# tier4/lidar_feature_extraction

Hardware: AMD Instinct MI355X
Metric: scans/sec (64-ring x 1800 synthetic scans, extraction hot path, inputs resident in HBM) (higher is better)
Workload: dtype f64

## Files before the change

lidar_feature_extraction_amd/csrc/lfx_kernels_unit.hpp:

```cpp
#pragma once

#include "lfx_kernels_common.hpp"

#pragma clang fp contract(off)

namespace lfx
{

enum { kBitLK, kBitJL, kBitJR, kBitA, kBitS, kBitSelE, kBitSelS, kUnitBitArrays };

template<int CH>
struct UnitLds
{
  static constexpr int kSpan = 64 * CH;
  static constexpr int kBitWords = 2 * (CH + 2);
  uint32_t bits[kUnitBitArrays][kBitWords];
  double r[kSpan];
  union {
    double c[kSpan + 2];
    float2 pxy[kSpan + 2];
  };
  static constexpr int kBaseDwords = (kSpan * 8 + (kSpan + 2) * 8 + kUnitBitArrays * kBitWords * 4) / 4;
  static constexpr int kMinPadDwords = 2 * (2 * CH - 2);
  static constexpr int kPadDwords = ((8 - kBaseDwords % 32) + 32) % 32 + (((8 - kBaseDwords % 32) + 32) % 32 < kMinPadDwords ? 32 : 0);
  uint32_t pad_[kPadDwords];
};
static_assert(sizeof(UnitLds<5>) % 128 == 32 && sizeof(UnitLds<3>) % 128 == 32 && sizeof(UnitLds<4>) % 128 == 32 &&
  sizeof(UnitLds<6>) % 128 == 32 && sizeof(UnitLds<12>) % 128 == 32, "slab stride");
static_assert(7 * 4 * sizeof(UnitLds<5>) <= 160 * 1024 && 6 * 4 * sizeof(UnitLds<6>) <= 160 * 1024 && 8 * 4 * sizeof(UnitLds<4>) <= 160 * 1024,
  "workgroups per CU the launch bounds count on");
#ifndef LFX_UNIT_WAVES_CH5
#define LFX_UNIT_WAVES_CH5 7
#endif
#ifndef LFX_LIBRARY_SQRT
#define LFX_LIBRARY_SQRT 0
#endif
#ifndef LFX_COS_BAND
#define LFX_COS_BAND 0x1p-20f
#endif
constexpr int unit_waves_per_simd(int ch, int variant = 0, bool xf = false)
{
  return ch > 6 ? 3 : (ch == 6 ? 5 : (ch == 5 ? (variant == 0 && !xf ? LFX_UNIT_WAVES_CH5 : 6) : (ch == 4 ? 7 : 8)));
}

#define LFX_WAVE_SYNC() \
  do { \
    __builtin_amdgcn_fence(__ATOMIC_RELEASE, "wavefront"); \
    __builtin_amdgcn_wave_barrier(); \
    __builtin_amdgcn_fence(__ATOMIC_ACQUIRE, "wavefront"); \
  } while (0)

template<int NW>
__device__ __forceinline__ void lds_window_f64(const double * first, double (&w)[NW])
{
  static_assert(NW <= 22, "extend the wait's operand list");
  const uint32_t addr = (uint32_t)reinterpret_cast<uintptr_t>(first);
#pragma unroll
  for (int i = 0; i < NW; i++) {
    asm volatile ("ds_read_b64 %0, %1 offset:%2" : "=v"(w[i]) : "v"(addr), "n"(8 * i));
  }
  if constexpr (NW == 2) {
    asm volatile ("s_waitcnt lgkmcnt(0)" : "+v"(w[0]), "+v"(w[1]));
  } else if constexpr (NW == 5) {
    asm volatile ("s_waitcnt lgkmcnt(0)" : "+v"(w[0]), "+v"(w[1]), "+v"(w[2]), "+v"(w[3]), "+v"(w[4]));
  } else if constexpr (NW == 11) {
// ... 84 lines not shown
    }
#undef LFX_WRITELANE
    static_assert(kUnitMaxChunks <= 12, "one case per chunk");
  }
};

template<int CH>
__device__ __forceinline__ void put_words(UnitLds<CH> & U, int arr, const WordVec & v, int lane)
{
  const uint32_t addr = (uint32_t)reinterpret_cast<uintptr_t>(&U.bits[arr][0]) + 8u * (uint32_t)lane;
  const uint64_t data = ((uint64_t)v.hi << 32) | v.lo;
  uint64_t saved;
  asm volatile ("s_mov_b64 %0, exec\n\ts_mov_b64 exec, %3\n\tds_write_b64 %1, %2\n\ts_mov_b64 exec, %0"
    : "=&s"(saved) : "v"(addr), "v"(data), "n"((1u << (CH + 2)) - 1u) : "memory");
}

template<int CH>
__device__ inline uint32_t get_win(const UnitLds<CH> & U, int arr, int k, const UnitWin & w)
{
  const u32_alias_t * b = reinterpret_cast<const u32_alias_t *>(&U.bits[arr][2 * k + w.ofs]);
  return __builtin_amdgcn_alignbit(b[1], b[0], w.sh);
}

template<int CH>
__device__ inline uint32_t get_win_at(const UnitLds<CH> & U, int arr, int first)
{
  const uint32_t bit = (uint32_t)(first + 64);
  const u32_alias_t * b = reinterpret_cast<const u32_alias_t *>(&U.bits[arr][bit >> 5]);
  return __builtin_amdgcn_alignbit(b[1], b[0], bit & 31u);
}

__device__ __forceinline__ uint32_t from_lane_below(uint32_t v) {return (uint32_t)__builtin_amdgcn_update_dpp(0, (int)v, 0x138, 0xF, 0xF, true);}
__device__ __forceinline__ uint32_t from_lane_above(uint32_t v) {return (uint32_t)__builtin_amdgcn_update_dpp(0, (int)v, 0x130, 0xF, 0xF, true);}

template<int CH, int PT>
__device__ __forceinline__ uint32_t row_frame(uint32_t own)
{
  static_assert(PT >= 1 && PT <= 2 * CH && (PT > CH ? 3 * CH + PT : 2 * CH + PT) <= 32,
    "the halo of a lane's positions must lie in the two lanes either side of it, the frame in one register");
  const uint32_t below = from_lane_below(own), above = from_lane_above(own);
  uint32_t f = (own << PT) | (above << (PT + CH));
  if constexpr (PT >= CH) {f |= below << (PT - CH);} else {f |= below >> (CH - PT);}
  if constexpr (PT > CH) {
    f |= from_lane_below(below) >> (2 * CH - PT);
    f |= from_lane_above(above) << (PT + 2 * CH);
  }
  return f;
}

template<int CH>
__device__ __forceinline__ uint32_t row_hits(uint32_t frame, const uint32_t (&mask)[CH])
{
  uint32_t h = 0;
#pragma unroll
  for (int d = 0; d < CH; d++) {
    const uint32_t t = frame & mask[d];
    h |= (t < 1u ? t : 1u) << d;
  }
  return h;
}

template<int CH> struct RowDiv { static constexpr uint32_t kShift = 18, kMul = ((1u << 18) + CH - 1) / CH; };
template<int CH> constexpr bool row_div_exact()
{
  for (uint32_t q = 0; q < 64u * CH; q++) {
    if (((q * RowDiv<CH>::kMul) >> RowDiv<CH>::kShift) != q / CH) {return false;}
// ... 61 lines not shown
struct OrgScan
{
  const uint8_t * __restrict__ pts;
  const uint32_t * __restrict__ scan_begin;
  uint32_t * __restrict__ ring_count_out;
  uint32_t R, r0, wave, drop_zero;
  const uint32_t * __restrict__ xform;
  const uint32_t * __restrict__ geom;
};

struct UnitGeom
{
  int N, b0, b1, o0, o1, g0, span, K, qb0, qb1, qo0, qo1, qlo, qhi;
};

__device__ inline UnitGeom unit_geometry(int N, int P, int B, int j, int b0, int b1)
{
  UnitGeom G;
  G.N = N; G.b0 = b0; G.b1 = b1;
  G.o0 = j == 0 ? 0 : b0; G.o1 = j == B - 1 ? N : b1;
  const int H = P + 1;
  G.g0 = G.o0 - H; G.span = G.o1 + H - G.g0;
  G.K = (G.span + 63) >> 6;
  G.qb0 = b0 - G.g0; G.qb1 = b1 - G.g0;
  G.qo0 = G.o0 - G.g0; G.qo1 = G.o1 - G.g0;
  G.qlo = G.g0 < 0 ? -G.g0 : 0;
  G.qhi = (N - G.g0) < G.span ? (N - G.g0) : G.span;
  return G;
}

template<int PT, int CH, bool DEF, bool ORG, bool XF, bool SIDX = false>
__device__ __forceinline__ uint32_t unit_core(
  const Params & prm, UnitLds<CH> & U, const UnitGeom & G, uint32_t dbg_flags, uint32_t s, uint32_t slot, int j,
  const float (&x)[CH], const float (&y)[CH], const float (&z)[CH], const uint32_t (&src)[CH],
  const UnitTables * __restrict__ tab, bool second_pass, const OrgScan & og, size_t off, uint32_t max_rings,
  uint32_t rec_lo, uint32_t rec_hi, uint32_t & n_edge, uint32_t & n_surface, const int lane)
{
  const int P = PT > 0 ? PT : prm.P, B = prm.B;
  (void)B;
  const int N = G.N, o0 = G.o0, o1 = G.o1, g0 = G.g0, span = G.span, K = G.K;
  const int qb0 = G.qb0, qb1 = G.qb1, qo0 = G.qo0, qo1 = G.qo1, qlo = G.qlo, qhi = G.qhi;
  (void)o0; (void)o1;
  const UnitWin W0{(uint32_t)(lane + 48) >> 5, (uint32_t)(lane + 16) & 31u};
  const UnitWin W1{(uint32_t)(lane + 49) >> 5, (uint32_t)(lane + 17) & 31u};
  constexpr uint32_t kOvrOccluded = 1u, kOvrRange = 2u, kOvrBeam = 4u;
  uint32_t ovr[(CH + 9) / 10];
#pragma unroll
  for (int t = 0; t < (CH + 9) / 10; t++) {ovr[t] = 0;}
  LFX_STAMP(2);
#pragma unroll
  for (int k = 0; k < CH; k++) {
    if (k < K) {
      const int q = 64 * k + lane;
      const double xd = (double)x[k], yd = (double)y[k];
      U.r[q] = sqrt_sum_of_squares(xd * xd + yd * yd);
    }
  }
  LFX_WAVE_SYNC();
  LFX_STAMP(3);
  {
    asm volatile ("" ::: "memory");
    const double dist_diff = DEF ? 0.3 : tab->prm.dist_diff;
    const double min_range = DEF ? 0.1 : tab->prm.min_range, max_range = DEF ? 100.0 : tab->prm.max_range;
    const double pb_ratio = DEF ? 0.02 : tab->prm.pb_ratio;
    const float pb_ratio_f = DEF ? 0.02f : tab->prm.pb_ratio_f;
    const double cos_bound = tab->prm.cos_bound;
    const int pair_end = qo1 < qhi - 1 ? qo1 : qhi - 1;
    uint64_t bad = 0;
    uint64_t zero_pair = 0;
    uint64_t prev_top = 0;
    WordVec vlk, vjl, vjr;
    const float cbf = tab->prm.cos_bound_f;
    const bool ratio_ok = pb_ratio_f >= 0x1p-9f;
    double c_dd = dist_diff, c_min = min_range, c_max = max_range;
    float c_one_lo = 1.0f - LFX_COS_BAND, c_one_hi = 1.0f + LFX_COS_BAND, c_tiny = 1e-18f, c_big = 1e30f, c_zero = 0.f, c_small = 1e-30f;
    asm volatile ("" : "+v"(c_dd), "+v"(c_min), "+v"(c_max), "+v"(c_one_lo), "+v"(c_one_hi), "+v"(c_tiny), "+v"(c_big), "+v"(c_zero), "+v"(c_small));
#pragma unroll
    for (int k = 0; k < CH; k++) {
      if (k < K) {
        const int q = 64 * k + lane;
        const uint64_t pair = in_span(q, qlo, qhi - 1);
        const float2 nb = U.pxy[q + 1];
        double rw3[3];
        lds_window_f64(&U.r[k == 0 ? (q > 0 ? q - 1 : 0) : q - 1], rw3);
        double rk = rw3[1], rn = rw3[2];
        const double rm = rw3[0];
        if (k == 0) {
          rk = q == 0 ? rw3[0] : rk;
          rn = q == 0 ? rw3[1] : rn;
        }
        zero_pair |= pair & in_span(q, qo0, qo1) & bal(rk == 0.) & bal(rn == 0.);
        {
          uint64_t spec;
          const uint64_t less = polar_less_masks(x[k], y[k], nb.x, nb.y, spec, c_tiny);
          bad |= in_span(q, qo0, pair_end) & (spec | ~less);
        }
        const float dotf = x[k] * nb.x + y[k] * nb.y;
        const float denf = (float)rk * (float)rn;
        const float cosf = dotf * __builtin_amdgcn_rcpf(denf);
        const uint64_t yes = bal(cosf > cbf + LFX_COS_BAND) & bal(cosf < c_one_lo);
        const uint64_t no = bal(cosf < cbf - LFX_COS_BAND) | bal(cosf > c_one_hi);
        const uint64_t fin = bal(denf > c_small) & bal(denf < c_big);
        uint64_t lk = yes & ~no & fin & pair;
        const uint64_t undecided = (~(yes | no) | ~fin) & pair;
        if (undecided != 0ull) {
          const double dot = (double)x[k] * (double)nb.x + (double)y[k] * (double)nb.y;
          const double cosang = dot / (rk * rn);
          lk |= undecided & bal(cosang >= cos_bound) & bal(cosang <= 1.0);
        }
        vlk.set(k, lk);
        const double rq = rk + c_dd;
        const uint64_t jl = lk & in_span(q, 0, N - P - 1 - g0) & bal(rn > rq);
        const uint64_t lk_prev = (lk << 1) | prev_top;
        const uint64_t jr = lk_prev & in_span(q, P + 1 - g0, qhi) & bal(rm > rq);
        prev_top = lk >> 63;
        if (LFX_STAGE_ON(256u)) {
          vjl.set(k, jl);
          vjr.set(k, jr);
        }
        uint64_t pb = 0;
        if (LFX_STAGE_ON(512u)) {
          const float rf = (float)rk, rmf = (float)rm, rpf = (float)rn;
          const float a1 = fabsf(rmf - rf), a2 = fabsf(rpf - rf);
          const float thr = pb_ratio_f * rf;
          const float hi_t = thr * (1.0f + 0x1p-12f), lo_t = thr * (1.0f - 0x1p-12f);
          const uint64_t guard = ratio_ok ? (bal(rf > c_zero) & bal(rf < c_big)) : 0ull;
          const uint64_t yy = bal(a1 > hi_t) & bal(a2 > hi_t) & guard;
          const uint64_t nn = (bal(a1 < lo_t) | bal(a2 < lo_t)) & guard;
          const uint64_t valid = in_span(q, 1 - g0, N - 1 - g0) & in_span(q, qo0, qo1);
          pb = yy & valid;
          const uint64_t undecided = valid & ~(yy | nn);
          if (undecided != 0ull) {
            const float ratio1 = (float)(fabs(rm - rk) / rk);
            const float ratio2 = (float)(fabs(rn - rk) / rk);
            pb |= undecided & bal((double)ratio1 > pb_ratio) & bal((double)ratio2 > pb_ratio);
          }
        }
        const uint64_t oor = ~(bal(c_min <= rk) & bal(rk <= c_max));
        ovr[k / 10] |= (lanes(oor) ? (uint32_t)kOvrRange << (3 * (k % 10)) : 0u) | (lanes(pb) ? (uint32_t)kOvrBeam << (3 * (k % 10)) : 0u);
      }
    }
    if (bad != 0ull) {
      bool really = false;
#pragma unroll
      for (int k = 0; k < CH; k++) {
        if (k < K) {
          const int q = 64 * k + lane;
          const bool pair = q >= qo0 && q < pair_end;
          const float2 nb = U.pxy[q + 1];
          if (pair && !polar_less(x[k], y[k], nb.x, nb.y)) {really = true;}
        }
      }
      if (__ballot(really) != 0ull) {return (uint32_t)(second_pass ? kDeferOther : kDeferOrder);}
    }
    if (zero_pair != 0ull) {return (uint32_t)kDeferOther;}
    put_words(U, kBitLK, vlk, lane);
    if (LFX_STAGE_ON(256u)) {
      put_words(U, kBitJL, vjl, lane);
      put_words(U, kBitJR, vjr, lane);
    }
  }
  LFX_STAMP(4);
  constexpr bool kRows = PT > 0 && PT <= 2 * CH && (CH <= 6 || (CH == 12 && PT <= 5));
  constexpr bool kRowPick = kRows;
  constexpr int kRowWin = kRows ? 2 * PT + CH : 1;
  constexpr int kSetStride = CH < 4 ? 4 : CH;
  const int p0 = CH * lane;
  uint32_t reach[CH];
  uint32_t rch[CH];
  uint32_t occ_rows = 0, own_rows = 0;
#pragma unroll
  for (int k = 0; k < (kRowPick ? 0 : CH); k++) {
    reach[k] = 0;
    if (k < K) {
      const int q = 64 * k + lane;
      const uint32_t lw = get_win(U, kBitLK, k, W0);
      int Lr = __clz((int)~(lw << 16));
      int Rr = __ffs((int)~(lw >> 16)) - 1;
      Lr = Lr < P ? Lr : P;
      Rr = Rr < P ? Rr : P;
      const uint32_t left = ((1u << (Lr + 1)) - 1u) << (15 - Lr);
      const uint32_t right = ((1u << (Rr + 1)) - 1u) << 16;
      if (LFX_STAGE_ON(256u)) {
        ovr[k / 10] |= ((get_win(U, kBitJL, k, W0) & left) | (get_win(U, kBitJR, k, W1) & right)) != 0u ? kOvrOccluded << (3 * (k % 10)) : 0u;
      }
      const int Lb = Lr < q - qb0 ? Lr : q - qb0;
      const int Rb = Rr < qb1 - 1 - q ? Rr : qb1 - 1 - q;
      reach[k] = lanes(in_span(q, qb0, qb1)) ? (((1u << (Lb + Rb + 1)) - 1u) << (16 - Lb)) : 0u;
    }
  }
  LFX_WAVE_SYNC();
  LFX_STAMP(5);
  const int row_base = p0 - PT;
  if constexpr (kRows) {
    double w[kRowWin];
    lds_window_f64(&U.r[row_base], w);
#pragma unroll
    for (int d = 0; d < CH; d++) {
      double sum = 0.;
#pragma unroll
      for (int t = 0; t <= 2 * PT; t++) {
        const double v = w[d + t];
        sum += (t == PT) ? v * (-2. * PT) : v;
      }
      const int width = qb1 - qb0;
      U.c[p0 + d] = (uint32_t)(p0 + d - qb0) < (uint32_t)(width > 0 ? width : 0) ? sum * sum : 0.;
    }
  }
#pragma unroll
  for (int k = 0; k < (kRows ? 0 : CH); k++) {
    if (k < K) {
      const int q = 64 * k + lane;
      int qq = q < P ? P : q;
      qq = qq > 64 * CH - 1 - P ? 64 * CH - 1 - P : qq;
      double sum = 0.;
      if (PT > 0 && 2 * PT + 1 <= 11) {
        double w[2 * (PT > 0 ? PT : 0) + 1];
        lds_window_f64(&U.r[qq - PT], w);
#pragma unroll
        for (int d = -(PT > 0 ? PT : 0); d <= (PT > 0 ? PT : 0); d++) {
          const double v = w[d + PT];
          sum += (d == 0) ? v * (-2. * PT) : v;
        }
      } else {
        for (int d = -P; d <= P; d++) {
          const double v = U.r[qq + d];
          sum += (d == 0) ? v * (-2. * P) : v;
        }
      }
      U.c[q] = lanes(in_span(q, qb0, qb1)) ? sum * sum : 0.;
    }
  }
  LFX_WAVE_SYNC();
  LFX_STAMP(6);
  asm volatile ("" ::: "memory");
  const double edge_thr = DEF ? 0.05 : tab->prm.edge_thr, surf_thr = DEF ? 0.05 : tab->prm.surf_thr;
  uint32_t lt[CH];
  uint64_t ecand[CH], scand[CH];
  constexpr uint32_t kEdgeCand = 1u << ((PT > 0 ? PT : 1) + 18), kSurfCand = 1u << ((PT > 0 ? PT : 1) + 17);
  if constexpr (kRowPick) {
    constexpr int PR = PT > 0 ? PT : 1;
    double w[kRowWin];
    lds_window_f64(&U.c[row_base], w);
    uint32_t ec = 0, sc = 0;
#pragma unroll
    for (int d = 0; d < CH; d++) {
      const double ci = w[d + PR];
      uint32_t m = 0;
#pragma unroll
      for (int t = PR; t >= 1; t--) {m = m + m + (uint32_t)(w[d + PR + t] < ci);}
      m = m + m;
#pragma unroll
      for (int t = 1; t <= PR; t++) {m = m + m + (uint32_t)(w[d + PR - t] <= ci);}
      lt[d] = m << d;
      ec |= (ci >= edge_thr ? 1u : 0u) << d;
      sc |= (ci <= surf_thr ? 1u : 0u) << d;
    }
    {
      constexpr int kFrame = CH + 2 * PR;
      const uint32_t LW = get_win_at(U, kBitLK, p0 - PR - 1);
      uint32_t JLW = 0, JRW = 0;
      if (LFX_STAGE_ON(256u)) {
        JLW = get_win_at(U, kBitJL, p0 - PR - 1);
// ... 13 lines not shown
        const uint32_t o = ((JLW << (32 - fj)) >> (31u - Lr)) | ((JRW >> (fj + 1)) << (31u - Rr));
        occ_rows |= (o < 1u ? o : 1u) << d;
        const uint32_t run = (((1u << (Lr + Rr + 1u)) - 1u) << ((uint32_t)fp - Lr)) & IB;
        rch[d] = ((IB >> fp) & 1u) != 0u ? run : 0u;
      }
    }
    LFX_STAMP(7);
    uint32_t hp[CH];
    auto pick_pass = [&](uint32_t live) -> uint32_t {
      uint32_t sel = 0;
      for (;; ) {
        const uint32_t pk = live & ~row_hits<CH>(row_frame<CH, PR>(live), hp);
        if (__builtin_amdgcn_ballot_w64(pk != 0u) == 0ull) {break;}
        sel |= pk;
        live &= ~row_hits<CH>(row_frame<CH, PR>(pk), rch);
        if (__builtin_amdgcn_ballot_w64(live != 0u) == 0ull) {break;}
      }
      return sel;
    };
    uint32_t sel_e = 0, sel_s = 0, by_e = 0, by_s = 0;
    if (LFX_STAGE_KEPT(1u)) {
#pragma unroll
      for (int d = 0; d < CH; d++) {hp[d] = ~lt[d] & rch[d] & ~(1u << (PR + d));}
      sel_e = pick_pass(ec & own_rows);
      by_e = row_hits<CH>(row_frame<CH, PR>(sel_e), rch);
    }
    LFX_STAMP(8);
    if (LFX_STAGE_KEPT(64u)) {
#pragma unroll
      for (int d = 0; d < CH; d++) {hp[d] = lt[d] & rch[d];}
      sel_s = pick_pass(sc & own_rows & ~by_e);
      by_s = row_hits<CH>(row_frame<CH, PR>(sel_s), rch);
    }
    if constexpr (5 * kSetStride <= 32) {
      reinterpret_cast<u32_alias_t *>(U.r)[lane] =
        by_e | by_s << kSetStride | sel_s << (2 * kSetStride) | sel_e << (3 * kSetStride) | occ_rows << (4 * kSetStride);
    } else {
      static_assert(5 * kSetStride <= 64, "the five sets of a lane share two words");
      reinterpret_cast<u64_alias_t *>(U.r)[lane] = (uint64_t)by_e | (uint64_t)by_s << kSetStride | (uint64_t)sel_s << (2 * kSetStride) |
        (uint64_t)sel_e << (3 * kSetStride) | (uint64_t)occ_rows << (4 * kSetStride);
    }
    LFX_WAVE_SYNC();
  } else {
#pragma unroll
    for (int k = 0; k < CH; k++) {
      lt[k] = 0;
      ecand[k] = 0; scand[k] = 0;
      if (k < K) {
        const int q = 64 * k + lane;
        int qc = q < P ? P : q;
        qc = qc > span - 1 - P ? span - 1 - P : qc;
        uint32_t m = 0;
        if (PT > 0 && 2 * PT + 1 <= 11) {
          double w[2 * (PT > 0 ? PT : 0) + 1];
          lds_window_f64(&U.c[qc - PT], w);
          const double ci = w[PT];
#pragma unroll
          for (int d = (PT > 0 ? PT : 1); d >= 1; d--) {m = m + m + (uint32_t)(w[PT + d] < ci);}
          m = m + m;
#pragma unroll
          for (int d = 1; d <= (PT > 0 ? PT : 1); d++) {m = m + m + (uint32_t)(w[PT - d] <= ci);}
          m <<= 16 - (PT > 0 ? PT : 1);
          m |= ci >= edge_thr ? kEdgeCand : 0u;
          m |= ci <= surf_thr ? kSurfCand : 0u;
        } else {
          const double ci = U.c[qc];
          for (int d = 1; d <= P; d++) {
            const double cl = U.c[qc - d], cr = U.c[qc + d];
            m |= (cl <= ci) ? (1u << (16 - d)) : 0u;
            m |= (cr < ci) ? (1u << (16 + d)) : 0u;
          }
          ecand[k] = bal(ci >= edge_thr);
// ... 65 lines not shown
          if ((S[k] | S[k + 1] | S[k + 2]) != 0ull) {
            A[k] &= ~bal((get_win(U, kBitS, k, W0) & reach[k]) != 0u);
            va.set(k, A[k]);
          }
          left |= A[k];
        }
      }
      if (left == 0ull) {break;}
      put_words(U, kBitA, va, lane);
    }
    {
      WordVec vsel;
#pragma unroll
      for (int k = 0; k < CH; k++) {
        if (k < K) {vsel.set(k, SEL[k]);}
      }
      put_words(U, sel_arr, vsel, lane);
    }
  }
  LFX_STAMP(9);
  uint32_t pe = 0, ps = 0;
  asm volatile ("" ::: "memory");
  uint8_t * __restrict__ label_s = tab->label_s;
  double * __restrict__ curv_s = tab->curv_s;
  auto final_label = [&](int k, int q) -> uint32_t {
    uint32_t l = kDefault;
    uint32_t t = (ovr[k / 10] >> (3 * (k % 10))) & 7u;
    if constexpr (kRowPick) {
      static_assert(row_div_exact<CH>(), "q / CH by multiplication");
      const uint32_t row = __umul24((uint32_t)q, RowDiv<CH>::kMul) >> RowDiv<CH>::kShift, d = (uint32_t)q - (uint32_t)CH * row;
      constexpr int S = kSetStride;
      uint32_t idx, occ_bit;
      if constexpr (5 * S > 32) {
        const uint64_t sets = reinterpret_cast<const u64_alias_t *>(U.r)[row] >> d;
        idx = ((uint32_t)sets & 1u) | ((uint32_t)(sets >> (S - 1)) & 2u) | ((uint32_t)(sets >> (2 * S - 2)) & 4u) | ((uint32_t)(sets >> (3 * S - 3)) & 8u);
        occ_bit = (uint32_t)(sets >> (4 * S)) & 1u;
      } else {
      const uint32_t sets = reinterpret_cast<const u32_alias_t *>(U.r)[row] >> d;
      constexpr uint32_t kFour = 1u | 1u << S | 1u << (2 * S) | 1u << (3 * S);
      constexpr uint32_t kGather = 1u | 1u << (S - 1) | 1u << (2 * (S - 1)) | 1u << (3 * (S - 1));
      idx = (__umul24(sets & kFour, kGather) >> (3 * (S - 1))) & 15u;
      occ_bit = (sets >> (4 * S)) & 1u;
      }
      constexpr auto block_label = [](uint32_t i) -> uint64_t {
        return (i & 8u) ? kEdge : ((i & 4u) ? kSurface : ((i & 2u) ? kSurfaceNeighbor : ((i & 1u) ? kEdgeNeighbor : kDefault)));
      };
      constexpr uint64_t kBlockLabel =
        block_label(0) | block_label(1) << 4 | block_label(2) << 8 | block_label(3) << 12 | block_label(4) << 16 | block_label(5) << 20 |
        block_label(6) << 24 | block_label(7) << 28 | block_label(8) << 32 | block_label(9) << 36 | block_label(10) << 40 |
        block_label(11) << 44 | block_label(12) << 48 | block_label(13) << 52 | block_label(14) << 56 | block_label(15) << 60;
      l = (uint32_t)(kBlockLabel >> (4u * idx)) & 7u;
      t |= occ_bit;
    } else {
      const uint32_t wE = get_win(U, kBitSelE, k, W0), wS = get_win(U, kBitSelS, k, W0);
      l = (wE & reach[k]) != 0u ? (uint32_t)kEdgeNeighbor : l;
      l = (wS & reach[k]) != 0u ? (uint32_t)kSurfaceNeighbor : l;
      l = (wS & (1u << 16)) != 0u ? (uint32_t)kSurface : l;
      l = (wE & (1u << 16)) != 0u ? (uint32_t)kEdge : l;
    }
    constexpr uint32_t kOverride = (uint32_t)kOccluded << 4 | (uint32_t)kOutOfRange << 8 | (uint32_t)kOutOfRange << 12 |
      (uint32_t)kParallelBeam << 16 | (uint32_t)kParallelBeam << 20 | (uint32_t)kParallelBeam << 24 | (uint32_t)kParallelBeam << 28;
    l = t != 0u ? (kOverride >> (4u * t)) & 15u : l;
    return lanes(in_span(q, qo0, qo1)) ? l : (uint32_t)kDefault;
  };
  typedef __attribute__((address_space(1))) uint8_t g_u8_t;
  typedef __attribute__((address_space(1))) double g_f64_t;
  typedef __attribute__((address_space(1))) uint32_t g_u32_t;
  typedef float f32x4_t __attribute__((ext_vector_type(4)));
  typedef __attribute__((address_space(1))) f32x4_t g_f32x4_t;
  g_u8_t * const label_u = (g_u8_t *)label_s + ((ptrdiff_t)off + g0);
  g_f64_t * const curv_u = (g_f64_t *)curv_s + ((ptrdiff_t)off + g0);
  g_f32x4_t * const rec_u = (g_f32x4_t *)tab->rec_pts + (off + rec_lo);
  g_u32_t * const idx_u = (g_u32_t *)tab->rec_idx + (off + rec_lo);
  g_u32_t * const sidx_u = SIDX ? (g_u32_t *)tab->sidx + ((ptrdiff_t)off + g0) : nullptr;
  (void)rec_hi;
  uint32_t lab[CH];
#pragma unroll
  for (int k = 0; k < CH; k++) {
    lab[k] = kDefault;
    if (k < K) {
      const int q = 64 * k + lane;
      const bool own = lanes(in_span(q, qo0, qo1));
      const uint32_t l = final_label(k, q);
      const double cv = U.c[q];
      if (own) {
        label_u[(uint32_t)q] = (uint8_t)l;
        if (curv_s != nullptr) {curv_u[(uint32_t)q] = cv;}
#ifndef LFX_WHATIF_NO_SIDX
        if constexpr (SIDX) {sidx_u[(uint32_t)q] = src[k];}
#endif
      }
      const uint64_t fe = bal(l == kEdge), fs = bal(l == kSurface);
      lab[k] = l;
      pe += __popcll(fe);
      ps += __popcll(fs);
    }
  }
  {
    if ((pe | ps) != 0u && LFX_STAGE_ON(1024u)) {
      constexpr uint32_t kRecSlot = rec_slot_places(PT, CH);
      static_assert(kRecBytes * kRecSlot <= 8 * 64 * CH, "the range slab stages a slot's records");
      LFX_WAVE_SYNC();
      f32x4_t * const stage_pts = reinterpret_cast<f32x4_t *>(U.r);
      u32_alias_t * const stage_idx = reinterpret_cast<u32_alias_t *>(stage_pts + kRecSlot);
      uint32_t re = 0, rs = pe;
#pragma unroll
      for (int k = 0; k < CH; k++) {
        if (k < K) {
          const uint64_t fe = bal(lab[k] == kEdge), fs = bal(lab[k] == kSurface);
          if ((fe | fs) != 0ull) {
            if (lanes(fe | fs)) {
              const int q = 64 * k + lane, i = g0 + q;
              const uint32_t be = __builtin_amdgcn_mbcnt_hi((uint32_t)(fe >> 32), __builtin_amdgcn_mbcnt_lo((uint32_t)fe, 0u));
              const uint32_t bs = __builtin_amdgcn_mbcnt_hi((uint32_t)(fs >> 32), __builtin_amdgcn_mbcnt_lo((uint32_t)fs, 0u));
              const uint32_t rank = lab[k] == kEdge ? re + be : rs + bs;
              const f32x4_t rec = {x[k], y[k], z[k], (float)U.c[q]};
              const uint32_t idx = ORG ? (XF ? ring_column(og.xform[s * kRings + slot], (uint32_t)i, (uint32_t)N) : (uint32_t)i) * og.R + slot : src[k];
              if (rank < kRecSlot) {
                stage_pts[rank] = rec;
                stage_idx[rank] = idx;
              } else {
                rec_u[rank] = rec;
                idx_u[rank] = idx;
              }
            }
            re += (uint32_t)__popcll(fe);
            rs += (uint32_t)__popcll(fs);
          }
        }
      }
      LFX_WAVE_SYNC();
      const uint32_t staged = pe + ps < kRecSlot ? pe + ps : kRecSlot;
      g_f32x4_t * const slot_pts = (g_f32x4_t *)tab->rec32 + ((((size_t)s * max_rings + slot) * (uint32_t)B + (uint32_t)j) * (kRecSlot * kRecBytes / 16u));
      g_u32_t * const slot_idx = reinterpret_cast<g_u32_t *>(slot_pts + staged);
#pragma unroll
      for (uint32_t r0 = 0; r0 < kRecSlot; r0 += 64) {
        const uint32_t r = r0 + (uint32_t)lane;
        if (r < staged) {
          slot_pts[r] = stage_pts[r];
          slot_idx[r] = stage_idx[r];
        }
      }
    }
  }
  LFX_STAMP(10);
  n_edge = pe;
  n_surface = ps;
  return 0u;
}
// ... 34 lines not shown
      if (lane == 0) {scan_falls_back(tab, s, (reason) == kDeferOrder ? (uint32_t)kScanOrderFell : 0u);} \
    } else if (lane == 0 && (atomicOr(tab->ring_flags + s * kRings + slot, (reason)) & kDeferMask) == 0u) { \
      defer_list[atomicAdd(defer_count, 1u)] = s * kRings + slot; \
    } \
    return; \
  } while (0)
  LFX_STAMP(0);
  if (N < 2 * P + 1 || N - 2 * P < B || (uint32_t)N > lds_ring_cap(ring_cap)) {
    if (j == 0) {LFX_DEFER(kDeferOther);}
    return;
  }
  int b0, b1;
  if (ORG) {
    b0 = org_b0;
    b1 = org_b1;
  } else {
    const int bj = block_boundary(N, P, B, j + (lane & 1));
    b0 = __builtin_amdgcn_readlane(bj, 0);
    b1 = __builtin_amdgcn_readlane(bj, 1);
  }
  const UnitGeom G = unit_geometry(N, P, B, j, b0, b1);
  if (b1 - b0 < 2 || G.span > (64 * CH)) {LFX_DEFER(kDeferOther);}
  const int o0 = G.o0, o1 = G.o1, g0 = G.g0, qlo = G.qlo, qhi = G.qhi;

  LFX_STAMP(1);
  {
    uint32_t * z = &U.bits[0][0];
    constexpr int kBitDwords = kUnitBitArrays * UnitLds<CH>::kBitWords;
#pragma unroll
    for (int w0 = 0; w0 < kBitDwords; w0 += 64) {
      if (w0 + 64 <= kBitDwords || lane + w0 < kBitDwords) {z[lane + w0] = 0u;}
    }
  }
  float x[CH], y[CH], z[CH];
  uint32_t src[CH];
  if (ORG) {
    const uint32_t sub = (uint32_t)lane & 3u, cq = (uint32_t)lane >> 2;
    const uint32_t rr = og.r0 + sub;
    const uint32_t rload = rr < og.R ? rr : og.R - 1u;
    float4 rec[CH];
    uint32_t rw[CH];
    const uint8_t * const base = og.pts + (size_t)scan_first * 32u;
    const uint32_t xf = XF ? og.xform[s * kRings + rload] : 0u;
#pragma unroll
    for (int m = 0; m < CH; m++) {
      const int q = 64 * m + 16 * (int)og.wave + (int)cq;
      int i = g0 + q;
      i = i < g0 + qlo ? g0 + qlo : (i > g0 + qhi - 1 ? g0 + qhi - 1 : i);
      const uint32_t col = XF ? ring_column(xf, (uint32_t)i, (uint32_t)N) : (uint32_t)i;
      const uint8_t * p = base + (col * og.R + rload) * 32u;
      rec[m] = *reinterpret_cast<const float4 *>(p);
      rw[m] = *reinterpret_cast<const uint32_t *>(p + 20);
    }
    __builtin_amdgcn_sched_barrier(0);
    uint64_t wrong = 0;
    uint32_t zero_seen = 0;
    f32_alias_t * zex = reinterpret_cast<f32_alias_t *>(slabs[sub].r);
#pragma unroll
    for (int m = 0; m < CH; m++) {
      const int q = 64 * m + 16 * (int)og.wave + (int)cq;
      const uint64_t in = in_span(q, qlo, qhi);
      uint64_t bad = bal((rw[m] & 0xFFFFu) != rr);
      if (og.drop_zero) {
        const uint64_t zb = bal(rec[m].x == 0.f) & bal(rec[m].y == 0.f) & bal(rec[m].z == 0.f);
        bad |= zb;
        zero_seen |= (zb & in) != 0ull ? 1u : 0u;
      }
      wrong |= bad & in;
      const bool inl = lanes(in);
      slabs[sub].pxy[q] = make_float2(inl ? rec[m].x : 0.f, inl ? rec[m].y : 0.f);
      zex[q] = rec[m].z;
    }
    wrong &= bal(rr < og.R);
    __syncthreads();
    if (wrong != 0ull) {
      if (zero_seen != 0u) {
        if (lane == 0) {scan_falls_back(tab, s, (uint32_t)kScanZeroFell);}
        return;
      }
      LFX_DEFER(kDeferOther);
    }
    if (slot >= og.R) {return;}
#pragma unroll
    for (int k = 0; k < CH; k++) {
      const int q = 64 * k + lane;
      const float2 v = U.pxy[q];
      x[k] = v.x; y[k] = v.y;
      z[k] = reinterpret_cast<const f32_alias_t *>(U.r)[q];
      src[k] = 0u;
    }
  } else {
    float2 v[CH];
#pragma unroll
    for (int k = 0; k < CH; k++) {
      const int q = 64 * k + lane;
      int i = g0 + q;
      i = i < 0 ? 0 : (i > N - 1 ? N - 1 : i);
      v[k] = sxy[off + i];
      z[k] = sz[off + i];
      src[k] = sidx[off + i];
    }
    __builtin_amdgcn_sched_barrier(0);
#pragma unroll
    for (int k = 0; k < CH; k++) {
      const int q = 64 * k + lane;
      const bool in = lanes(in_span(q, qlo, qhi));
      x[k] = in ? v[k].x : 0.f;
      y[k] = in ? v[k].y : 0.f;
      U.pxy[q] = make_float2(x[k], y[k]);
    }
  }
  LFX_WAVE_SYNC();
  uint32_t pe = 0, ps = 0;
  {
    const uint32_t why = unit_core<PT, CH, DEF, ORG, XF>(prm, U, G, dbg_flags, s, slot, j, x, y, z, src, tab, second_pass, og, off, max_rings,
      (uint32_t)o0, (uint32_t)o1, pe, ps, lane);
    if (why != 0u) {LFX_DEFER(why);}
  }
  if (lane == 0) {
    const size_t ui = ((size_t)s * kRings + slot) * kUnitMaxBlocks + j;
    tab->unit_ne[ui] = pe;
    tab->unit_ns[ui] = ps;
    tab->unit_span[ui] = kUnitRecordsInSlot | ((uint32_t)o1 << 16) | (uint32_t)o0;
    if (ORG) {
      (void)__hip_atomic_fetch_add(tab->ring_nedge + s * kRings + slot, pe, __ATOMIC_RELAXED, __HIP_MEMORY_SCOPE_AGENT);
      (void)__hip_atomic_fetch_add(tab->ring_nsurf + s * kRings + slot, ps, __ATOMIC_RELAXED, __HIP_MEMORY_SCOPE_AGENT);
    }
    if (j == 0) {
      tab->ring_status[s * kRings + slot] = kOk;
      if (ORG) {
        og.ring_count_out[s * kRings + slot] = (uint32_t)N;
        if (slot == 0) {
          tab->scan_info[s * 4 + kInfoRings] = og.R;
          atomicOr(tab->scan_flags + s, (uint32_t)kScanFused);
        }
      }
    }
  }
#undef LFX_DEFER
}

template<int PT, int CH, bool DEF>
__device__ __forceinline__ void unit_body_holes(
  const Params & prm, UnitLds<CH> * __restrict__ slabs, uint32_t ring_cap, uint32_t max_rings, uint32_t dbg_flags, uint32_t s,
  uint32_t slot, int j, const UnitTables * __restrict__ tab, const OrgScan & og)
{
  constexpr int kLoads = holes_loads(CH);
  constexpr int kQv = (kLoads + 3) / 4;
  const int lane = threadIdx.x & 63;
  const uint32_t w = og.wave;
  UnitLds<CH> & U = slabs[w];
  const int P = PT > 0 ? PT : prm.P, B = prm.B;
  const uint32_t sub = (uint32_t)lane & 3u, cq = (uint32_t)lane >> 2;
  const uint32_t rr = og.r0 + sub, rload = rr < og.R ? rr : og.R - 1u;
  const uint32_t scan_first = og.scan_begin[s];
  const uint32_t C = og.geom[s * kGeomStride];
  const uint32_t flags = tab->scan_flags[s];
  const uint16_t * __restrict__ cum16 = tab->cum16;
  const uint4 * __restrict__ dsc = tab->hole_desc + ((size_t)s * og.R) * (uint32_t)B + (uint32_t)j;
  uint4 d[4];
#pragma unroll
  for (int r = 0; r < 4; r++) {
    const uint32_t ring = og.r0 + (uint32_t)r < og.R ? og.r0 + (uint32_t)r : og.R - 1u;
    d[r] = dsc[(size_t)ring * (uint32_t)B];
  }
  asm volatile ("" :: "s"(scan_first), "s"(C), "s"(flags), "s"(d[0].x), "s"(d[1].x), "s"(d[2].x), "s"(d[3].x));
  if (C == 0u || (flags & kScanCountFell) != 0u) {return;}
  const uint32_t stride = cum_stride(ring_cap);
  const int n_pieces = (int)((C + kPieceCols - 1u) / kPieceCols);
  LFX_STAMP(0);
  int pstart = 0x7FFFFFFF, pend = -1;
  int N_l = 0, b0_l = 0, b1_l = 0;
  bool dead_l = true;
#pragma unroll
  for (int r = 0; r < 4; r++) {
    const bool dead_r = og.r0 + (uint32_t)r >= og.R || ((d[r].y >> 16) & kHoleUnitDead) != 0u;
    if (!dead_r) {
      const int ps = (int)(d[r].z & 0xFFFFu), pe = (int)(d[r].z >> 16);
      pstart = ps < pstart ? ps : pstart;
      pend = pe > pend ? pe : pend;
    }
    if (sub == (uint32_t)r) {
      N_l = (int)(d[r].x & 0xFFFFu); b0_l = (int)(d[r].x >> 16); b1_l = (int)(d[r].y & 0xFFFFu);
      dead_l = dead_r;
    }
  }
  const int o0_l = j == 0 ? 0 : b0_l, o1_l = j == B - 1 ? N_l : b1_l;
// ... 2 lines not shown
  const int N = __builtin_amdgcn_readlane(N_l, (int)w);
  const bool dead = __builtin_amdgcn_readlane((int)dead_l, (int)w) != 0;
  const int n_need = pend - pstart + 1;
  if (n_need <= 0 || n_need > 4 * kLoads) {return;}
  LFX_STAMP(13);
  uint32_t qv[kQv];
  {
    const uint16_t * row = cum16 + ((size_t)s * og.R + rload) * stride;
#pragma unroll
    for (int v = 0; v < kQv; v++) {
      const int e = pstart + 16 * v + (int)cq;
      qv[v] = row[e < n_pieces ? e : n_pieces];
    }
  }
  float4 rec[kLoads];
  const uint8_t * const base = og.pts + (size_t)scan_first * 32u + (size_t)rload * 32u;
#pragma unroll
  for (int m = 0; m < kLoads; m++) {
    const int t = 4 * m + (int)w;
    const uint32_t col = (uint32_t)(pstart + t) * kPieceCols + cq;
    rec[m] = make_float4(0.f, 0.f, 0.f, 0.f);
    if (t < n_need && col < C) {rec[m] = *reinterpret_cast<const float4 *>(base + (size_t)col * og.R * 32u);}
  }
  {
    uint32_t * zb = &U.bits[0][0];
    constexpr int kBitDwords = kUnitBitArrays * UnitLds<CH>::kBitWords;
#pragma unroll
    for (int w0 = 0; w0 < kBitDwords; w0 += 64) {
      if (w0 + 64 <= kBitDwords || lane + w0 < kBitDwords) {zb[lane + w0] = 0u;}
    }
  }
  __builtin_amdgcn_sched_barrier(0);
  {
    f32_alias_t * zex = reinterpret_cast<f32_alias_t *>(slabs[sub].r);
    u32_alias_t * cex = reinterpret_cast<u32_alias_t *>(slabs[sub].r) + 64 * CH;
    const uint64_t ring_lanes = 0x1111111111111111ull << sub;
#pragma unroll
    for (int m = 0; m < kLoads; m++) {
      const int t = 4 * m + (int)w;
      const uint32_t col = (uint32_t)(pstart + t) * kPieceCols + cq;
      const bool valid = t < n_need && col < C && !dead_l && !(rec[m].x == 0.f && rec[m].y == 0.f && rec[m].z == 0.f);
      const uint64_t vm = bal(valid) & ring_lanes;
      const uint32_t rank = __builtin_amdgcn_mbcnt_hi((uint32_t)(vm >> 32), __builtin_amdgcn_mbcnt_lo((uint32_t)vm, 0u));
      const uint32_t before = (uint32_t)__shfl((int)qv[(t >> 4) < kQv ? (t >> 4) : kQv - 1], 4 * (t & 15) + (int)sub);
      const int q = (int)(before + rank) - g0_l;
      if (valid && (uint32_t)q < (uint32_t)(64 * CH)) {
        slabs[sub].pxy[q] = make_float2(rec[m].x, rec[m].y);
        zex[q] = rec[m].z;
        cex[q] = col;
      }
    }
  }
  LFX_STAMP(14);
  __syncthreads();
  if (dead) {return;}
  const int b0 = __builtin_amdgcn_readlane(b0_l, (int)w), b1 = __builtin_amdgcn_readlane(b1_l, (int)w);
  const UnitGeom G = unit_geometry(N, P, B, j, b0, b1);
  const int o0 = G.o0, o1 = G.o1, qlo = G.qlo, qhi = G.qhi;
  const size_t off = ring_base(s, slot, max_rings, ring_cap);
  LFX_STAMP(1);
  float x[CH], y[CH], z[CH];
  uint32_t src[CH];
#pragma unroll
  for (int k = 0; k < CH; k++) {
    const int q = 64 * k + lane;
    const bool in = lanes(in_span(q, qlo, qhi));
    const float2 v = U.pxy[q];
    x[k] = in ? v.x : 0.f; y[k] = in ? v.y : 0.f;
    z[k] = reinterpret_cast<const f32_alias_t *>(U.r)[q];
    src[k] = reinterpret_cast<const u32_alias_t *>(U.r)[64 * CH + q] * og.R + slot;
  }
  LFX_WAVE_SYNC();
#pragma unroll
  for (int k = 0; k < CH; k++) {
    const int q = 64 * k + lane;
    if (!lanes(in_span(q, qlo, qhi))) {U.pxy[q] = make_float2(0.f, 0.f);}
  }
  LFX_WAVE_SYNC();
  uint32_t pe = 0, ps = 0;
  {
    const uint32_t why = unit_core<PT, CH, DEF, false, false, true>(prm, U, G, dbg_flags, s, slot, j, x, y, z, src, tab, false, og, off, max_rings,
      (uint32_t)o0, (uint32_t)o1, pe, ps, lane);
    if (why != 0u) {
      if (lane == 0) {scan_falls_back(tab, s, why == kDeferOrder ? (uint32_t)kScanOrderFell : 0u);}
      return;
    }
  }
  if (lane == 0) {
    const size_t ui = ((size_t)s * kRings + slot) * kUnitMaxBlocks + j;
    tab->unit_ne[ui] = pe;
    tab->unit_ns[ui] = ps;
    tab->unit_span[ui] = kUnitRecordsInSlot | ((uint32_t)o1 << 16) | (uint32_t)o0;
    (void)__hip_atomic_fetch_add(tab->ring_nedge + s * kRings + slot, pe, __ATOMIC_RELAXED, __HIP_MEMORY_SCOPE_AGENT);
    (void)__hip_atomic_fetch_add(tab->ring_nsurf + s * kRings + slot, ps, __ATOMIC_RELAXED, __HIP_MEMORY_SCOPE_AGENT);
    if (j == 0) {tab->ring_status[s * kRings + slot] = kOk;}
  }
}

template<int V> struct UnitVariant
{
  static constexpr int kPT = V <= 1 ? 5 : (V == 2 ? 2 : 0);
  static constexpr bool kDEF = V == 0;
};

constexpr int unit_list_waves_per_simd(int ch, int variant, bool loop)
{
  const int w = unit_waves_per_simd(ch, variant, true) - (variant == 2 && ch >= 5 ? 1 : 0);
  return loop ? (w > 4 ? (w - 3 < 4 ? w - 3 : 4) : (w > 1 ? w - 1 : 1)) : w;
}
template<int V, bool SECOND, int CH, bool LOOP = false>
__global__ __launch_bounds__(64 * kUnitWaves, unit_list_waves_per_simd(CH, V, LOOP)) void ring_unit_kernel(
  Params prm, uint32_t ring_cap, uint32_t dbg_flags, uint32_t max_rings, const uint32_t * __restrict__ ring_count,
  const float2 * __restrict__ sxy, const float * __restrict__ sz,
  const uint32_t * __restrict__ sidx, const UnitTables * __restrict__ tab,
// ... 75 lines not shown
```

Measured before the change: 906,700.

## Shrink per-wave LDS slab by aliasing range, curvature and positions to fit eight waves

The per-wave LDS slab now overlays the range, curvature and xy arrays in one union and adds a separate float z array. Neighbour positions are taken from registers through DPP and readlane instead of LDS, and curvature is buffered in registers before being written over the shared storage. The smaller slab lets the CH=5 variant raise its waves per SIMD from seven to eight. The cost is extra register pressure from the cc and cf arrays and a new shared cols array, and the reuse of aliased storage adds ordering hazards that the wave syncs must cover.

```diff
diff --git a/lidar_feature_extraction_amd/csrc/lfx_kernels_unit.hpp b/lidar_feature_extraction_amd/csrc/lfx_kernels_unit.hpp
--- a/lidar_feature_extraction_amd/csrc/lfx_kernels_unit.hpp
+++ b/lidar_feature_extraction_amd/csrc/lfx_kernels_unit.hpp
@@ -15,22 +15,22 @@
   static constexpr int kSpan = 64 * CH;
   static constexpr int kBitWords = 2 * (CH + 2);
   uint32_t bits[kUnitBitArrays][kBitWords];
-  double r[kSpan];
   union {
-    double c[kSpan + 2];
-    float2 pxy[kSpan + 2];
+    double r[kSpan];
+    double c[kSpan];
+    float2 pxy[kSpan];
   };
-  static constexpr int kBaseDwords = (kSpan * 8 + (kSpan + 2) * 8 + kUnitBitArrays * kBitWords * 4) / 4;
-  static constexpr int kMinPadDwords = 2 * (2 * CH - 2);
-  static constexpr int kPadDwords = ((8 - kBaseDwords % 32) + 32) % 32 + (((8 - kBaseDwords % 32) + 32) % 32 < kMinPadDwords ? 32 : 0);
+  float z[kSpan];
+  static constexpr int kBaseDwords = (kSpan * 8 + kSpan * 4 + kUnitBitArrays * kBitWords * 4) / 4;
+  static constexpr int kPadDwords = ((8 - kBaseDwords % 32) + 32) % 32;
   uint32_t pad_[kPadDwords];
 };
 static_assert(sizeof(UnitLds<5>) % 128 == 32 && sizeof(UnitLds<3>) % 128 == 32 && sizeof(UnitLds<4>) % 128 == 32 &&
   sizeof(UnitLds<6>) % 128 == 32 && sizeof(UnitLds<12>) % 128 == 32, "slab stride");
-static_assert(7 * 4 * sizeof(UnitLds<5>) <= 160 * 1024 && 6 * 4 * sizeof(UnitLds<6>) <= 160 * 1024 && 8 * 4 * sizeof(UnitLds<4>) <= 160 * 1024,
+static_assert(8 * 4 * sizeof(UnitLds<5>) <= 160 * 1024 && 6 * 4 * sizeof(UnitLds<6>) <= 160 * 1024 && 8 * 4 * sizeof(UnitLds<4>) <= 160 * 1024,
   "workgroups per CU the launch bounds count on");
 #ifndef LFX_UNIT_WAVES_CH5
-#define LFX_UNIT_WAVES_CH5 7
+#define LFX_UNIT_WAVES_CH5 8
 #endif
 #ifndef LFX_LIBRARY_SQRT
 #define LFX_LIBRARY_SQRT 0
@@ -181,6 +181,13 @@
 
 __device__ __forceinline__ uint32_t from_lane_below(uint32_t v) {return (uint32_t)__builtin_amdgcn_update_dpp(0, (int)v, 0x138, 0xF, 0xF, true);}
 __device__ __forceinline__ uint32_t from_lane_above(uint32_t v) {return (uint32_t)__builtin_amdgcn_update_dpp(0, (int)v, 0x130, 0xF, 0xF, true);}
+
+template<int CH>
+__device__ __forceinline__ float next_position(const float (&v)[CH], int k)
+{
+  const int first_of_next = k + 1 < CH ? __builtin_amdgcn_readlane(__float_as_int(v[k + 1 < CH ? k + 1 : k]), 0) : 0;
+  return __int_as_float(__builtin_amdgcn_update_dpp(first_of_next, __float_as_int(v[k]), 0x130, 0xF, 0xF, false));
+}
 
 template<int CH, int PT>
 __device__ __forceinline__ uint32_t row_frame(uint32_t own)
@@ -308,7 +315,7 @@
 template<int PT, int CH, bool DEF, bool ORG, bool XF, bool SIDX = false>
 __device__ __forceinline__ uint32_t unit_core(
   const Params & prm, UnitLds<CH> & U, const UnitGeom & G, uint32_t dbg_flags, uint32_t s, uint32_t slot, int j,
-  const float (&x)[CH], const float (&y)[CH], const float (&z)[CH], const uint32_t (&src)[CH],
+  const float (&x)[CH], const float (&y)[CH], const uint32_t (&src)[CH],
   const UnitTables * __restrict__ tab, bool second_pass, const OrgScan & og, size_t off, uint32_t max_rings,
   uint32_t rec_lo, uint32_t rec_hi, uint32_t & n_edge, uint32_t & n_surface, const int lane)
 {
@@ -356,7 +363,7 @@
       if (k < K) {
         const int q = 64 * k + lane;
         const uint64_t pair = in_span(q, qlo, qhi - 1);
-        const float2 nb = U.pxy[q + 1];
+        const float2 nb = make_float2(next_position(x, k), next_position(y, k));
         double rw3[3];
         lds_window_f64(&U.r[k == 0 ? (q > 0 ? q - 1 : 0) : q - 1], rw3);
         double rk = rw3[1], rn = rw3[2];
@@ -423,7 +430,7 @@
         if (k < K) {
           const int q = 64 * k + lane;
           const bool pair = q >= qo0 && q < pair_end;
-          const float2 nb = U.pxy[q + 1];
+          const float2 nb = make_float2(next_position(x, k), next_position(y, k));
           if (pair && !polar_less(x[k], y[k], nb.x, nb.y)) {really = true;}
         }
       }
@@ -483,6 +490,7 @@
       U.c[p0 + d] = (uint32_t)(p0 + d - qb0) < (uint32_t)(width > 0 ? width : 0) ? sum * sum : 0.;
     }
   }
+  double cc[kRows ? 1 : CH];
 #pragma unroll
   for (int k = 0; k < (kRows ? 0 : CH); k++) {
     if (k < K) {
@@ -504,7 +512,14 @@
           sum += (d == 0) ? v * (-2. * P) : v;
         }
       }
-      U.c[q] = lanes(in_span(q, qb0, qb1)) ? sum * sum : 0.;
+      cc[k] = lanes(in_span(q, qb0, qb1)) ? sum * sum : 0.;
+    }
+  }
+  if constexpr (!kRows) {
+    LFX_WAVE_SYNC();
+#pragma unroll
+    for (int k = 0; k < CH; k++) {
+      if (k < K) {U.c[64 * k + lane] = cc[k];}
     }
   }
   LFX_WAVE_SYNC();
@@ -584,12 +599,13 @@
       sel_s = pick_pass(sc & own_rows & ~by_e);
       by_s = row_hits<CH>(row_frame<CH, PR>(sel_s), rch);
     }
+    static_assert(sizeof(U.bits) >= 64 * (5 * kSetStride <= 32 ? 4 : 8), "the bit arrays hold the labelling words");
     if constexpr (5 * kSetStride <= 32) {
-      reinterpret_cast<u32_alias_t *>(U.r)[lane] =
+      reinterpret_cast<u32_alias_t *>(U.bits)[lane] =
         by_e | by_s << kSetStride | sel_s << (2 * kSetStride) | sel_e << (3 * kSetStride) | occ_rows << (4 * kSetStride);
     } else {
       static_assert(5 * kSetStride <= 64, "the five sets of a lane share two words");
-      reinterpret_cast<u64_alias_t *>(U.r)[lane] = (uint64_t)by_e | (uint64_t)by_s << kSetStride | (uint64_t)sel_s << (2 * kSetStride) |
+      reinterpret_cast<u64_alias_t *>(U.bits)[lane] = (uint64_t)by_e | (uint64_t)by_s << kSetStride | (uint64_t)sel_s << (2 * kSetStride) |
         (uint64_t)sel_e << (3 * kSetStride) | (uint64_t)occ_rows << (4 * kSetStride);
     }
     LFX_WAVE_SYNC();
@@ -721,11 +737,11 @@
       constexpr int S = kSetStride;
       uint32_t idx, occ_bit;
       if constexpr (5 * S > 32) {
-        const uint64_t sets = reinterpret_cast<const u64_alias_t *>(U.r)[row] >> d;
+        const uint64_t sets = reinterpret_cast<const u64_alias_t *>(U.bits)[row] >> d;
         idx = ((uint32_t)sets & 1u) | ((uint32_t)(sets >> (S - 1)) & 2u) | ((uint32_t)(sets >> (2 * S - 2)) & 4u) | ((uint32_t)(sets >> (3 * S - 3)) & 8u);
         occ_bit = (uint32_t)(sets >> (4 * S)) & 1u;
       } else {
-      const uint32_t sets = reinterpret_cast<const u32_alias_t *>(U.r)[row] >> d;
+      const uint32_t sets = reinterpret_cast<const u32_alias_t *>(U.bits)[row] >> d;
       constexpr uint32_t kFour = 1u | 1u << S | 1u << (2 * S) | 1u << (3 * S);
       constexpr uint32_t kGather = 1u | 1u << (S - 1) | 1u << (2 * (S - 1)) | 1u << (3 * (S - 1));
       idx = (__umul24(sets & kFour, kGather) >> (3 * (S - 1))) & 15u;
@@ -764,9 +780,11 @@
   g_u32_t * const sidx_u = SIDX ? (g_u32_t *)tab->sidx + ((ptrdiff_t)off + g0) : nullptr;
   (void)rec_hi;
   uint32_t lab[CH];
+  float cf[CH];
 #pragma unroll
   for (int k = 0; k < CH; k++) {
     lab[k] = kDefault;
+    cf[k] = 0.f;
     if (k < K) {
       const int q = 64 * k + lane;
       const bool own = lanes(in_span(q, qo0, qo1));
@@ -781,6 +799,7 @@
       }
       const uint64_t fe = bal(l == kEdge), fs = bal(l == kSurface);
       lab[k] = l;
+      cf[k] = (float)cv;
       pe += __popcll(fe);
       ps += __popcll(fs);
     }
@@ -788,7 +807,7 @@
   {
     if ((pe | ps) != 0u && LFX_STAGE_ON(1024u)) {
       constexpr uint32_t kRecSlot = rec_slot_places(PT, CH);
-      static_assert(kRecBytes * kRecSlot <= 8 * 64 * CH, "the range slab stages a slot's records");
+      static_assert(kRecBytes * kRecSlot <= 8 * 64 * CH, "the curvature slab stages a slot's records");
       LFX_WAVE_SYNC();
       f32x4_t * const stage_pts = reinterpret_cast<f32x4_t *>(U.r);
       u32_alias_t * const stage_idx = reinterpret_cast<u32_alias_t *>(stage_pts + kRecSlot);
@@ -803,7 +822,7 @@
               const uint32_t be = __builtin_amdgcn_mbcnt_hi((uint32_t)(fe >> 32), __builtin_amdgcn_mbcnt_lo((uint32_t)fe, 0u));
               const uint32_t bs = __builtin_amdgcn_mbcnt_hi((uint32_t)(fs >> 32), __builtin_amdgcn_mbcnt_lo((uint32_t)fs, 0u));
               const uint32_t rank = lab[k] == kEdge ? re + be : rs + bs;
-              const f32x4_t rec = {x[k], y[k], z[k], (float)U.c[q]};
+              const f32x4_t rec = {x[k], y[k], U.z[q], cf[k]};
               const uint32_t idx = ORG ? (XF ? ring_column(og.xform[s * kRings + slot], (uint32_t)i, (uint32_t)N) : (uint32_t)i) * og.R + slot : src[k];
               if (rank < kRecSlot) {
                 stage_pts[rank] = rec;
@@ -904,7 +923,7 @@
       if (w0 + 64 <= kBitDwords || lane + w0 < kBitDwords) {z[lane + w0] = 0u;}
     }
   }
-  float x[CH], y[CH], z[CH];
+  float x[CH], y[CH];
   uint32_t src[CH];
   if (ORG) {
     const uint32_t sub = (uint32_t)lane & 3u, cq = (uint32_t)lane >> 2;
@@ -927,7 +946,6 @@
     __builtin_amdgcn_sched_barrier(0);
     uint64_t wrong = 0;
     uint32_t zero_seen = 0;
-    f32_alias_t * zex = reinterpret_cast<f32_alias_t *>(slabs[sub].r);
 #pragma unroll
     for (int m = 0; m < CH; m++) {
       const int q = 64 * m + 16 * (int)og.wave + (int)cq;
@@ -941,7 +959,7 @@
       wrong |= bad & in;
       const bool inl = lanes(in);
       slabs[sub].pxy[q] = make_float2(inl ? rec[m].x : 0.f, inl ? rec[m].y : 0.f);
-      zex[q] = rec[m].z;
+      slabs[sub].z[q] = rec[m].z;
     }
     wrong &= bal(rr < og.R);
     __syncthreads();
@@ -958,11 +976,11 @@
       const int q = 64 * k + lane;
       const float2 v = U.pxy[q];
       x[k] = v.x; y[k] = v.y;
-      z[k] = reinterpret_cast<const f32_alias_t *>(U.r)[q];
       src[k] = 0u;
     }
   } else {
     float2 v[CH];
+    float z[CH];
 #pragma unroll
     for (int k = 0; k < CH; k++) {
       const int q = 64 * k + lane;
@@ -979,13 +997,13 @@
       const bool in = lanes(in_span(q, qlo, qhi));
       x[k] = in ? v[k].x : 0.f;
       y[k] = in ? v[k].y : 0.f;
-      U.pxy[q] = make_float2(x[k], y[k]);
+      U.z[q] = z[k];
     }
   }
   LFX_WAVE_SYNC();
   uint32_t pe = 0, ps = 0;
   {
-    const uint32_t why = unit_core<PT, CH, DEF, ORG, XF>(prm, U, G, dbg_flags, s, slot, j, x, y, z, src, tab, second_pass, og, off, max_rings,
+    const uint32_t why = unit_core<PT, CH, DEF, ORG, XF>(prm, U, G, dbg_flags, s, slot, j, x, y, src, tab, second_pass, og, off, max_rings,
       (uint32_t)o0, (uint32_t)o1, pe, ps, lane);
     if (why != 0u) {LFX_DEFER(why);}
   }
@@ -1025,6 +1043,7 @@
   const int P = PT > 0 ? PT : prm.P, B = prm.B;
   const uint32_t sub = (uint32_t)lane & 3u, cq = (uint32_t)lane >> 2;
   const uint32_t rr = og.r0 + sub, rload = rr < og.R ? rr : og.R - 1u;
+  __shared__ uint32_t cols[kUnitWaves][64 * CH + 8];
   const uint32_t scan_first = og.scan_begin[s];
   const uint32_t C = og.geom[s * kGeomStride];
   const uint32_t flags = tab->scan_flags[s];
@@ -1093,8 +1112,6 @@
   }
   __builtin_amdgcn_sched_barrier(0);
   {
-    f32_alias_t * zex = reinterpret_cast<f32_alias_t *>(slabs[sub].r);
-    u32_alias_t * cex = reinterpret_cast<u32_alias_t *>(slabs[sub].r) + 64 * CH;
     const uint64_t ring_lanes = 0x1111111111111111ull << sub;
 #pragma unroll
     for (int m = 0; m < kLoads; m++) {
@@ -1107,8 +1124,8 @@
       const int q = (int)(before + rank) - g0_l;
       if (valid && (uint32_t)q < (uint32_t)(64 * CH)) {
         slabs[sub].pxy[q] = make_float2(rec[m].x, rec[m].y);
-        zex[q] = rec[m].z;
-        cex[q] = col;
+        slabs[sub].z[q] = rec[m].z;
+        cols[sub][q] = col;
       }
     }
   }
@@ -1120,7 +1137,7 @@
   const int o0 = G.o0, o1 = G.o1, qlo = G.qlo, qhi = G.qhi;
   const size_t off = ring_base(s, slot, max_rings, ring_cap);
   LFX_STAMP(1);
-  float x[CH], y[CH], z[CH];
+  float x[CH], y[CH];
   uint32_t src[CH];
 #pragma unroll
   for (int k = 0; k < CH; k++) {
@@ -1128,19 +1145,12 @@
     const bool in = lanes(in_span(q, qlo, qhi));
     const float2 v = U.pxy[q];
     x[k] = in ? v.x : 0.f; y[k] = in ? v.y : 0.f;
-    z[k] = reinterpret_cast<const f32_alias_t *>(U.r)[q];
-    src[k] = reinterpret_cast<const u32_alias_t *>(U.r)[64 * CH + q] * og.R + slot;
-  }
-  LFX_WAVE_SYNC();
-#pragma unroll
-  for (int k = 0; k < CH; k++) {
-    const int q = 64 * k + lane;
-    if (!lanes(in_span(q, qlo, qhi))) {U.pxy[q] = make_float2(0.f, 0.f);}
+    src[k] = cols[w][q] * og.R + slot;
   }
   LFX_WAVE_SYNC();
   uint32_t pe = 0, ps = 0;
   {
-    const uint32_t why = unit_core<PT, CH, DEF, false, false, true>(prm, U, G, dbg_flags, s, slot, j, x, y, z, src, tab, false, og, off, max_rings,
+    const uint32_t why = unit_core<PT, CH, DEF, false, false, true>(prm, U, G, dbg_flags, s, slot, j, x, y, src, tab, false, og, off, max_rings,
       (uint32_t)o0, (uint32_t)o1, pe, ps, lane);
     if (why != 0u) {
       if (lane == 0) {scan_falls_back(tab, s, why == kDeferOrder ? (uint32_t)kScanOrderFell : 0u);}
```

Result: no change. 898,400 (median of 6 runs) (-0.9%).
